# nreHieW/Eagle

Hardware: AMD Instinct MI355X
Metric: frames/sec end-to-end (detect+keypoint+homography) @1280x720 (higher is better)
Workload: dtype f32 (split: hi/lo binary16 pairs, 3 x fp16 MFMA per product, fp32 accumulate); detector (1.4 % of the FLOP): f32, exact v_mfma_f32_16x16x4_f32 chains

## Files before the change

### eagle_amd/csrc/conv.hip

```cpp
#include <algorithm>
#include <cmath>
#include <cstdlib>
#include <mutex>

#include "common.h"
#include "dmath.h"
#include "conv_internal.h"

namespace eagle {

static int f16_ps(int kc) { const int g = kc / 8; return kc * 2 + ((g % 2 == 0) ? 16 : 0); }
static int f16_ni(int ks, int kc) { return (ks * ks * (kc / 8) + 3) / 4; }

enum FormKind { GENERIC, WSTAT, ADIRECT };
enum StrideForm { S1, S2D, S2T };
enum WeightImage { W_F32, W_F16, W_F16_S2D, W_SPLIT, W_SPLIT_AD, W_SPLIT_S2D, W_SPLIT_M32 };
struct Form {
    int prec, variant, kind;
    int pw;
    int sform, rows, cols;
    int kc, nt, halo_bufs;
    int wimage;
    int grid_cap;
    ConvKernelGetter get;
};
static constexpr Form gen(int prec, int variant, int pw, int wimage, int kind = GENERIC) { return {prec, variant, kind, pw, S1, 0, 0, 0, 0, 0, wimage, 0, nullptr}; }
static constexpr Form ad(int prec, int variant, int sform, int rows, int cols, int nt, int halo_bufs, int wimage, ConvKernelGetter get, int grid_cap = 0)
{
    return {prec, variant, ADIRECT, 0, sform, rows, cols, prec == EAGLE_PREC_F16 ? 32 : 16, nt, halo_bufs, wimage, grid_cap, get};
}
static constexpr int F16 = EAGLE_PREC_F16, F32 = EAGLE_PREC_F32, F32S = EAGLE_PREC_F32S;
static constexpr Form g_forms[] = {
    gen(F32, 0, 4, W_F32), gen(F32, 3, 2, W_F32), gen(F32, 4, 1, W_F32),
    gen(F16, 0, 4, W_F16), gen(F16, 2, 4, W_F16), gen(F16, 3, 2, W_F16), gen(F16, 4, 1, W_F16), gen(F16, 6, 4, W_F16, WSTAT), gen(F16, 7, 2, W_F16, WSTAT),
    ad(F16, 8, S1, 4, 32, 12, 2, W_F16, conv_ad_kernel_s1_bn192), ad(F16, 9, S1, 8, 32, 6, 2, W_F16, conv_ad_kernel_s1_bn96),
    ad(F16, 10, S2D, 4, 32, 12, 2, W_F16_S2D, conv_ad_kernel_s2_bn192), ad(F16, 11, S2D, 8, 32, 6, 2, W_F16_S2D, conv_ad_kernel_s2_bn96),
    gen(F32S, 0, 4, W_SPLIT), gen(F32S, 3, 2, W_SPLIT), gen(F32S, 18, 6, W_SPLIT),
    ad(F32S, 8, S1, 4, 32, 12, 2, W_SPLIT_AD, conv_ad_split_kernel_bn192), ad(F32S, 9, S1, 8, 32, 6, 2, W_SPLIT_AD, conv_ad_split_kernel_bn96),
    ad(F32S, 10, S2D, 4, 32, 12, 2, W_SPLIT_S2D, conv_ad_split_kernel_s2_bn192), ad(F32S, 11, S2D, 8, 32, 6, 2, W_SPLIT_S2D, conv_ad_split_kernel_s2_bn96),
    ad(F32S, 12, S1, 8, 32, 3, 2, W_SPLIT_AD, conv_ad_split_kernel48), ad(F32S, 13, S1, 16, 32, 3, 1, W_SPLIT_AD, conv_ad_split_kernel48sb),
    ad(F32S, 19, S1, 16, 32, 3, 2, W_SPLIT_AD, conv_ad_split_kernel48ring, 256),
    ad(F32S, 14, S2T, 4, 32, 12, 1, W_SPLIT_AD, conv_ad_split_kernel_s2t_bn192), ad(F32S, 15, S2T, 4, 32, 6, 1, W_SPLIT_AD, conv_ad_split_kernel_s2t_bn96),
    ad(F32S, 21, S1, 4, 32, 12, 2, W_SPLIT_M32, conv_ad_split32_kernel_bn192), ad(F32S, 22, S1, 8, 32, 6, 2, W_SPLIT_M32, conv_ad_split32_kernel_bn96),
    ad(F32S, 23, S1, 2, 64, 12, 2, W_SPLIT_M32, conv_ad_split32_kernel_w64_bn192), ad(F32S, 24, S1, 4, 64, 6, 2, W_SPLIT_M32, conv_ad_split32_kernel_w64_bn96)};

static const Form* find_form(int precision, int variant)
{
    for (const Form& f : g_forms)
        if (f.prec == precision && f.variant == variant) return &f;
    return nullptr;
}
static const Form& form_of(int precision, const ConvConfig& c)
{
    const Form* f = find_form(precision, c.variant);
    if (!f) fail(EAGLE_E_NOKERNEL, "no conv kernel form: prec=%d variant=%d", precision, c.variant);
    return *f;
}
static int kind_of(int precision, const ConvConfig& c) { const Form* f = find_form(precision, c.variant); return f ? f->kind : -1; }

static size_t lds_bytes(int precision, const ConvConfig& c)
{
    const Form& f = form_of(precision, c);
    if (f.kind == ADIRECT) {
        int hpix, rec, strips;
        if (precision == EAGLE_PREC_F16) { hpix = f.sform == S2D ? (f.rows + 1) * 33 : (f.rows + 2) * 34; rec = 96; strips = 4 * 32 * 112; }
        else if (f.wimage == W_SPLIT_M32) { hpix = (f.rows + 2) * (f.cols + 2); rec = 80; strips = 4 * 32 * 128; }
        else { hpix = f.sform == S2T ? (2 * f.rows + 1) * 66 : (f.rows + 2) * 34; rec = 96; strips = 4 * 16 * 208; }
        const int slabs = ((hpix * rec + 1023) / 1024 + 3) / 4 * 4;
        return (size_t)f.halo_bufs * slabs * 1024 + strips;
    }
    const int th = 4 * f.pw / c.wx, tw = 16 * c.wx;
    const int hw = (tw - 1) * c.stride + c.ks, hh = (th - 1) * c.stride + c.ks;
    const int bn = c.nt * 16;
    if (precision == EAGLE_PREC_F16) {
        const size_t operands = (size_t)f16_ni(c.ks, c.kc) * 4 * bn * 16 + (size_t)hh * hw * f16_ps(c.kc);
        const size_t strips = (size_t)4 * f.pw * 16 * (bn * 2 + 16);
        return f.kind == WSTAT ? operands + strips + 16 : std::max(operands + 16, strips);
    }
    if (precision == EAGLE_PREC_F32S) {
        const size_t operands = (size_t)f16_ni(c.ks, c.kc) * 2 * 4 * bn * 16 + (size_t)hh * hw * f16_ps(2 * c.kc);
        const size_t strips = (size_t)4 * f.pw * 16 * (bn * 4 + 16);
        return std::max(operands + 16, strips);
    }
    return (size_t)c.ks * c.ks * (c.kc / 4) * 4 * bn * 4 + (size_t)hh * hw * (c.kc + 1) * 4;
}

size_t conv_lds_bytes(int precision, const ConvConfig& c) { return lds_bytes(precision, c); }
int conv_tiles_per_frame(int precision, const ConvConfig& c, int ho, int wo)
{
    const Form& f = form_of(precision, c);
    const int th = f.kind == ADIRECT ? f.rows : 4 * f.pw / c.wx, tw = f.kind == ADIRECT ? f.cols : 16 * c.wx;
    return ((wo + tw - 1) / tw) * ((ho + th - 1) / th);
}

static const Inst* generic_inst(int precision, const ConvConfig& c)
{
    for (auto part : {conv_inst_part0, conv_inst_part1, conv_inst_part2, conv_inst_part3, conv_inst_split0, conv_inst_split1, conv_inst_split2}) {
        int n = 0;
        const Inst* t = part(&n);
        for (int k = 0; k < n; ++k)
            if (t[k].prec == precision && t[k].ks == c.ks && t[k].s == c.stride && t[k].kc == c.kc && t[k].nt == c.nt && t[k].variant == c.variant) return &t[k];
    }
    return nullptr;
}
bool conv_supported(int precision, const ConvConfig& c)
{
    const Form* f = find_form(precision, c.variant);
    if (f && f->kind == ADIRECT) return c.ks == 3 && c.stride == (f->sform == S1 ? 1 : 2) && c.kc == f->kc && c.nt == f->nt;
    return f && generic_inst(precision, c);
}

struct Tuned { int ks, s, cin, cout, wo, kc, nt, wx, variant; };
static const Tuned g_tuned[] = {
#include "conv_tuned.inc"
    {0, 0, 0, 0, 0, 0, 0, 0, 0}};
static const Tuned g_tuned_f32[] = {
#include "conv_tuned_f32.inc"
    {0, 0, 0, 0, 0, 0, 0, 0, 0}};
static const Tuned g_tuned_split[] = {
#include "conv_tuned_split.inc"
    {0, 0, 0, 0, 0, 0, 0, 0, 0}};
static bool tuned_match(const Tuned& t, const ConvConfig& c, int wo, ConvConfig* q)
{
    if (t.ks != c.ks || t.s != c.stride || t.cin != c.cin || t.cout != c.cout_pad || t.wo != wo) return false;
    *q = c; q->kc = t.kc; q->nt = t.nt; q->wx = t.wx; q->variant = t.variant;
    return true;
}

static bool env_force(const char* name, int* a, int* b, int* c) { const char* f = getenv(name); return f && sscanf(f, "%d,%d,%d", a, b, c) == 3; }
static bool env_off(const char* name) { const char* e = getenv(name); return e && atoi(e) == 0; }

static const int g_nts[] = {6, 4, 3, 2, 1};
static ConvConfig with_ad(ConvConfig c, int kc, int v192, int v96)
{
    c.kc = kc;
    if (c.cout_pad % 192 == 0) { c.nt = 12; c.variant = v192; } else { c.nt = 6; c.variant = v96; }
    return c;
}

static ConvConfig choose_f32(ConvConfig c, int wo)
{
    ConvConfig q = c; q.kc = (c.cin < 16) ? 4 : 16;
    if (env_force("EAGLE_F32_FORCE", &q.nt, &q.wx, &q.variant) && (q.wx == 1 || q.wx == 2) && q.nt >= 1 && c.cout_pad % (16 * q.nt) == 0 &&
        conv_supported(EAGLE_PREC_F32, q) && lds_bytes(EAGLE_PREC_F32, q) <= 160 * 1024)
        return q;
    for (const Tuned& t : g_tuned_f32)
        if (tuned_match(t, c, wo, &q) && conv_supported(EAGLE_PREC_F32, q)) return q;
    c.nt = 1;
    for (int nt : g_nts)
        if (c.cout_pad % (16 * nt) == 0) { c.nt = nt; break; }
    c.kc = (c.cin < 16) ? 4 : 16;
    if (c.stride == 2 && c.ks == 3) {
        q = c; q.variant = 3;
        if (conv_supported(EAGLE_PREC_F32, q)) return q;
    }
    return c;
}

static ConvConfig choose_split(ConvConfig c, int wo, bool plain_epilogue)
{
    const int prec = EAGLE_PREC_F32S, cin = c.cin, cout = c.cout_pad;
    ConvConfig q = c;
    if (env_force("EAGLE_CONV_FORCE", &q.kc, &q.nt, &q.variant) && cin % q.kc == 0 && cout % (16 * q.nt) == 0 && conv_supported(prec, q)) {
        if (form_of(prec, q).pw == 6) q.wx = 3;
        if (lds_bytes(prec, q) <= 160 * 1024) return q;
    }
    if (plain_epilogue && c.ks == 3 && c.stride == 2 && cin % 48 == 0 && cout % 96 == 0) return with_ad(c, 16, 14, 15);
    if (!env_off("EAGLE_CONV_M32") && plain_epilogue && c.ks == 3 && c.stride == 1 && cin % 16 == 0 && cout % 96 == 0) return with_ad(c, 16, 21, wo > 32 ? 24 : 22);
    for (const Tuned& t : g_tuned_split)
        if (tuned_match(t, c, wo, &q)) {
            const Form* f = find_form(prec, q.variant);
            if (kind_of(prec, q) == ADIRECT && !(plain_epilogue && cin % (f->sform == S2D ? 16 : 48) == 0)) continue;
            if (conv_supported(prec, q) && lds_bytes(prec, q) <= 160 * 1024) return q;
        }
    if (plain_epilogue && c.ks == 3 && c.stride == 1 && cin % 48 == 0 && cout % 96 == 0) return with_ad(c, 16, 8, 9);
    static const int skcs[] = {32, 16, 8};
    long best = -1;
    c.nt = 1; c.kc = 8; c.variant = 0;
    for (int variant : {0, 3})
        for (int nt : g_nts) {
            if (cout % (16 * nt)) continue;
            for (int kc : skcs) {
                if (cin % kc) continue;
                ConvConfig t = c; t.nt = nt; t.kc = kc; t.variant = variant;
                if (!conv_supported(prec, t)) continue;
                if (lds_bytes(prec, t) > 80 * 1024) continue;
                const int pw = form_of(prec, t).pw;
                if (nt * pw > 12) continue;
                const long score = (long)nt * pw * 1000 + kc * 10 + (variant == 0 ? 1 : 0);
                if (score > best) { best = score; c.nt = nt; c.kc = kc; c.variant = variant; }
            }
        }
    return c;
}

static ConvConfig choose_f16(ConvConfig c, int wo, bool plain_epilogue, bool plain_one)
{
    const int prec = EAGLE_PREC_F16, cin = c.cin, cout = c.cout_pad;
    ConvConfig q = c;
    if (env_force("EAGLE_CONV_FORCE", &q.kc, &q.nt, &q.variant) && cin % q.kc == 0 && cout % (16 * q.nt) == 0 && conv_supported(prec, q) &&
        lds_bytes(prec, q) <= 160 * 1024 && (kind_of(prec, q) == WSTAT ? plain_one : kind_of(prec, q) == ADIRECT ? plain_epilogue : true))
        return q;
    if (plain_epilogue && c.ks == 3 && c.stride == 1 && cin % 32 == 0 && cout % 96 == 0) return with_ad(c, 32, 8, 9);
    if (plain_epilogue && c.ks == 3 && c.stride == 2 && cin % 8 == 0 && cin >= 32 && cout % 96 == 0) return with_ad(c, 32, 10, 11);
    for (const Tuned& t : g_tuned)
        if (tuned_match(t, c, wo, &q)) {
            if (kind_of(prec, q) == WSTAT && !plain_one) continue;
            if (conv_supported(prec, q) && lds_bytes(prec, q) <= 160 * 1024) return q;
        }
    static const int kcs[] = {64, 48, 32, 16, 8};
    long best = -1;
    c.nt = 1; c.kc = 8;
    for (int nt : g_nts) {
        if (cout % (16 * nt)) continue;
        for (int kc : kcs) {
            if (cin % kc) continue;
            ConvConfig t = c; t.nt = nt; t.kc = kc;
            if (!conv_supported(prec, t)) continue;
            if (lds_bytes(prec, t) > 80 * 1024) continue;
            const long score = (long)kc * nt * 1000 + kc;
            if (score > best) { best = score; c.nt = nt; c.kc = kc; }
        }
    }
    return c;
}

ConvConfig conv_choose(int precision, int ks, int stride, int cin_pad, int cout_pad, int wo, bool plain_epilogue, bool second_residual)
{
    ConvConfig c;
    c.ks = ks; c.stride = stride; c.cin = cin_pad; c.cout_pad = cout_pad;
    c.wx = (wo > 16) ? 2 : 1;
    if (precision == EAGLE_PREC_F32) return choose_f32(c, wo);
    if (precision == EAGLE_PREC_F32S) return choose_split(c, wo, plain_epilogue);
    return choose_f16(c, wo, plain_epilogue, plain_epilogue && !second_residual);
}

size_t conv_weight_elems(int precision, const ConvConfig& c)
{
    const int bn = c.nt * 16, nblk = c.cout_pad / bn, nch = c.cin / c.kc;
    switch (form_of(precision, c).wimage) {
    case W_F16_S2D: return (size_t)nblk * (4 * c.cin / 32) * 16 * bn * 8;
    case W_F16: return (size_t)nblk * nch * f16_ni(c.ks, c.kc) * 4 * bn * 8;
    case W_SPLIT_S2D: return (size_t)nblk * (4 * c.cin / 16) * 6 * 4 * bn * 8;
    case W_SPLIT_M32: return (size_t)nblk * (c.cin / 16) * 18 * (bn / 32) * 512;
    case W_SPLIT_AD: return (size_t)nblk * (c.cin / 16) * 14 * 4 * bn * 8;
    case W_SPLIT: return (size_t)nblk * nch * f16_ni(c.ks, c.kc) * 2 * 4 * bn * 8;
    default: return (size_t)nblk * nch * c.ks * c.ks * (c.kc / 4) * 4 * bn;
    }
}

void conv_tile_weights(int precision, const ConvConfig& c, const float* w, int cin_real, int cout_real, void* dst, float* descale)
{
    const int bn = c.nt * 16, nblk = c.cout_pad / bn, nch = c.cin / c.kc, taps = c.ks * c.ks, wimage = form_of(precision, c).wimage;
    auto W = [&](int tap, int ci, int co) -> float {
        return (ci < cin_real && co < cout_real) ? w[((size_t)tap * cin_real + ci) * cout_real + co] : 0.0f;
    };
    if (descale) *descale = 1.0f;
    if (precision == EAGLE_PREC_F32S) {
        float amax = 0.f;
        for (size_t k = 0; k < (size_t)taps * cin_real * cout_real; ++k) amax = std::max(amax, std::fabs(w[k]));
        int e = 0;
        if (amax > 0.f) (void)std::frexp(amax, &e);
        const int sw = 15 - e;
        const float scale = std::ldexp(1.0f, sw);
        if (descale) *descale = std::ldexp(1.0f, -(sw + 4));
        _Float16* d = (_Float16*)dst;
        if (wimage == W_SPLIT_S2D) {
            const int per_phase = c.cin / 16;
            for (int b = 0; b < nblk; ++b)
                for (int ch = 0; ch < 4 * per_phase; ++ch)
                    for (int k = 0; k < 6; ++k)
                        for (int qq = 0; qq < 4; ++qq)
                            for (int nn = 0; nn < bn; ++nn)
                                for (int j = 0; j < 8; ++j) {
                                    const int ph = ch / per_phase, c0 = (ch - ph * per_phase) * 16, ry = ph >> 1, rx = ph & 1;
                                    const int tp = k < 4 ? k : 2 * (k - 4) + (qq >> 1), tyy = tp >> 1, txx = tp & 1;
                                    const int ky = tyy == 0 ? (ry == 1 ? 0 : -1) : (ry == 0 ? 1 : 2), kx = txx == 0 ? (rx == 1 ? 0 : -1) : (rx == 0 ? 1 : 2);
                                    float v = 0.f;
                                    if (ky >= 0 && kx >= 0) v = W(ky * 3 + kx, c0 + (qq & 1) * 8 + j, b * bn + nn) * scale;
                                    const _Float16 hi = (_Float16)v;
                                    *d++ = k < 4 ? hi : (_Float16)(v - (float)hi);
                                }
            return;
        }
        if (wimage == W_SPLIT_M32) {
            for (int b = 0; b < nblk; ++b)
                for (int ch = 0; ch < c.cin / 16; ++ch)
                    for (int tap = 0; tap < 9; ++tap)
                        for (int part = 0; part < 2; ++part)
                            for (int mb = 0; mb < bn / 32; ++mb)
                                for (int l = 0; l < 64; ++l)
                                    for (int j = 0; j < 8; ++j) {
                                        const float v = W(tap, ch * 16 + (l >> 5) * 8 + j, b * bn + mb * 32 + (l & 31)) * scale;
                                        const _Float16 hi = (_Float16)v;
                                        *d++ = part == 0 ? hi : (_Float16)(v - (float)hi);
                                    }
            return;
        }
        if (wimage == W_SPLIT_AD) {
            for (int b = 0; b < nblk; ++b)
                for (int ch = 0; ch < c.cin / 16; ++ch)
                    for (int k = 0; k < 14; ++k)
                        for (int qq = 0; qq < 4; ++qq)
                            for (int nn = 0; nn < bn; ++nn)
                                for (int j = 0; j < 8; ++j) {
                                    const int tap = k < 9 ? k : 2 * (k - 9) + (qq >> 1);
                                    float v = 0.f;
                                    if (tap < 9) v = W(tap, ch * 16 + (qq & 1) * 8 + j, b * bn + nn) * scale;
                                    const _Float16 hi = (_Float16)v;
                                    *d++ = k < 9 ? hi : (_Float16)(v - (float)hi);
                                }
            return;
        }
        const int G = c.kc / 8, NGR = taps * G, NI = f16_ni(c.ks, c.kc);
        for (int b = 0; b < nblk; ++b)
            for (int ch = 0; ch < nch; ++ch)
                for (int i = 0; i < NI; ++i)
                    for (int part = 0; part < 2; ++part)
                        for (int qq = 0; qq < 4; ++qq)
                            for (int nn = 0; nn < bn; ++nn)
                                for (int j = 0; j < 8; ++j) {
                                    const int g = 4 * i + qq;
                                    float v = 0.f;
                                    if (g < NGR) { const int tap = g / G, cg = g % G; v = W(tap, ch * c.kc + cg * 8 + j, b * bn + nn) * scale; }
                                    const _Float16 hi = (_Float16)v;
                                    *d++ = part == 0 ? hi : (_Float16)(v - (float)hi);
                                }
        return;
    }
    if (wimage == W_F16_S2D) {
        _Float16* d = (_Float16*)dst;
        const int nch2 = 4 * c.cin / 32;
        for (int b = 0; b < nblk; ++b)
            for (int ch = 0; ch < nch2; ++ch)
                for (int g = 0; g < 16; ++g)
                    for (int nn = 0; nn < bn; ++nn)
                        for (int j = 0; j < 8; ++j) {
                            const int tp = g / 4, cg = g % 4, tyy = tp >> 1, txx = tp & 1;
                            const int sc = ch * 32 + cg * 8 + j, ph = sc / c.cin, ci = sc - ph * c.cin, ry = ph >> 1, rx = ph & 1;
                            const int ky = tyy == 0 ? (ry == 1 ? 0 : -1) : (ry == 0 ? 1 : 2), kx = txx == 0 ? (rx == 1 ? 0 : -1) : (rx == 0 ? 1 : 2);
                            *d++ = (_Float16)((ky < 0 || kx < 0) ? 0.f : W(ky * 3 + kx, ci, b * bn + nn));
                        }
        return;
    }
    if (precision == EAGLE_PREC_F16) {
        const int G = c.kc / 8, NGR = taps * G, NI = f16_ni(c.ks, c.kc);
        _Float16* d = (_Float16*)dst;
        for (int b = 0; b < nblk; ++b)
            for (int ch = 0; ch < nch; ++ch)
                for (int g = 0; g < NI * 4; ++g)
                    for (int nn = 0; nn < bn; ++nn)
                        for (int j = 0; j < 8; ++j) {
                            float v = 0.f;
                            if (g < NGR) {
                                const int tap = g / G, cg = g % G;
                                v = W(tap, ch * c.kc + cg * 8 + j, b * bn + nn);
                            }
                            *d++ = (_Float16)v;
                        }
    } else {
        const int CSTEPS = c.kc / 4;
        float* d = (float*)dst;
        for (int b = 0; b < nblk; ++b)
            for (int ch = 0; ch < nch; ++ch)
                for (int tap = 0; tap < taps; ++tap)
                    for (int cs = 0; cs < CSTEPS; ++cs)
                        for (int qq = 0; qq < 4; ++qq)
                            for (int nn = 0; nn < bn; ++nn) *d++ = W(tap, ch * c.kc + cs * 4 + qq, b * bn + nn);
    }
}

static std::mutex g_page_mutex;
static const void* conv_zero_page()
{
    static void* z[64] = {};
    int dev = 0;
    HIP_CHECK(hipGetDevice(&dev));
    std::lock_guard<std::mutex> g(g_page_mutex);
    if (!z[dev]) { HIP_CHECK(hipMalloc(&z[dev], 256)); HIP_CHECK(hipMemset(z[dev], 0, 256)); }
    return z[dev];
}
static void* conv_trash_page()
{
    static void* z[64] = {};
    int dev = 0;
    HIP_CHECK(hipGetDevice(&dev));
    std::lock_guard<std::mutex> g(g_page_mutex);
    if (!z[dev]) HIP_CHECK(hipMalloc(&z[dev], 8192));
    return z[dev];
}

void conv_launch(int precision, const ConvLaunch& L, hipStream_t s)
{
    const ConvConfig& c = L.cfg;
    if (!conv_supported(precision, c)) fail(EAGLE_E_NOKERNEL, "no conv kernel instance: prec=%d ks=%d s=%d kc=%d nt=%d", precision, c.ks, c.stride, c.kc, c.nt);
    const Form& f = form_of(precision, c);
    ConvArgs a;
    a.x = L.x.p; a.xcs = L.x.cs; a.xoff = L.x.off; a.N = L.x.n; a.H = L.x.h; a.W = L.x.w;
    a.w = L.w; a.bias = L.bias;
    a.y = L.y.p; a.ycs = L.y.cs; a.yoff = L.y.off; a.Ho = L.y.h; a.Wo = L.y.w;
    a.r1 = L.r1.p; a.r1cs = L.r1.cs; a.r1off = L.r1.off;
    a.r2 = L.r2.p; a.r2cs = L.r2.cs; a.r2off = L.r2.off;
    a.descale = L.descale;
    if (precision == EAGLE_PREC_F32S) {
        if (L.x.f32 != 2 || (L.r1.p && L.r1.f32 != 2) || (L.r2.p && L.r2.f32 != 2) || L.y.f32 != (L.out_f32 ? 1 : 2))
            fail(EAGLE_E_INVALID, "split conv: operand tensor formats do not match the family");
        a.xcs *= 2; a.xoff *= 2; a.r1cs *= 2; a.r1off *= 2; a.r2cs *= 2; a.r2off *= 2;
        if (!L.out_f32) { a.ycs *= 2; a.yoff *= 2; }
    }
    if (!a.r1 && a.r2) { a.r1 = a.r2; a.r1cs = a.r2cs; a.r1off = a.r2off; a.r2 = nullptr; }
    a.pre_act = L.pre_act; a.post_act = L.post_act; a.out_f32 = L.out_f32 || precision == EAGLE_PREC_F32;
    a.wx = c.wx;
    a.nchunks = c.cin / c.kc;
    a.zeros = conv_zero_page(); a.trash = conv_trash_page(); a.xcd = 0; a.gy = 1; a.stack = 0;
    a.am = L.am_slot ? *L.am_slot : nullptr; a.am_cs = c.cout_pad;
    a.sat = (L.sat_slot && precision == EAGLE_PREC_F32S) ? *L.sat_slot : nullptr;
    if (f.kind == ADIRECT) {
        if (a.out_f32 || a.pre_act != 0 || a.post_act > 1 || L.am_slot || (precision == EAGLE_PREC_F32S && c.cin % (f.wimage == W_SPLIT_AD ? 48 : 16)))
            fail(EAGLE_E_NOKERNEL, "A-direct conv needs 2-byte / split output, pre_act none, post_act in {none, ReLU} and, in the split family, Cin = 16 k (48 k for variants 8, 9 and 12 - 15)");
        if (f.sform == S2D) a.nchunks = 4 * c.cin / c.kc;
        a.tiles_x = (a.Wo + f.cols - 1) / f.cols; a.tiles_y = (a.Ho + f.rows - 1) / f.rows;
        a.gy = c.cout_pad / (c.nt * 16);
        const size_t lim = (size_t)1 << 31;
        if ((size_t)a.N * a.H * a.W * a.xcs * 2 >= lim || (size_t)a.N * a.Ho * a.Wo * std::max(std::max(a.ycs, a.r1 ? a.r1cs : 0), a.r2 ? a.r2cs : 0) * 2 >= lim)
            fail(EAGLE_E_INVALID, "fp16 conv: a tensor of %d frames reaches 2 GiB; use a smaller device batch", a.N);
        const int nres = (a.r1 ? 1 : 0) + (a.r2 ? 1 : 0);
        const int items = a.tiles_x * a.tiles_y * a.N * a.gy;
        const bool deep = items <= 256;
        for (bool d : {false, true}) ensure_max_dynamic_lds((const void*)f.get(nres, d), 160 * 1024);
        hipLaunchKernelGGL(f.get(nres, deep), dim3(f.grid_cap ? std::min(items, f.grid_cap) : items), dim3(256), lds_bytes(precision, c), s, a);
        HIP_CHECK(hipGetLastError());
        return;
    }
    const int th = 4 * f.pw / c.wx, tw = 16 * c.wx;
    a.tiles_x = (a.Wo + tw - 1) / tw; a.tiles_y = (a.Ho + th - 1) / th;
    if (precision == EAGLE_PREC_F32) {
        if (!env_off("EAGLE_F32_STACK") && c.stride == 1 && a.N > 1 && a.Ho == a.H) { a.stack = 1; a.tiles_y = (a.N * (a.Ho + 1) + th - 1) / th; }
        if ((size_t)a.N * a.H * a.W * a.xcs * 4 >= ((size_t)1 << 31)) fail(EAGLE_E_INVALID, "fp32 conv: the input tensor of %d frames reaches 2 GiB; use a smaller device batch", a.N);
    }
    const bool ws = f.kind == WSTAT;
    if (a.am && (!prec_is_f16_kernels(precision) || ws))
        fail(EAGLE_E_NOKERNEL, "fused heat-map maxima need the generic fp16 kernel");
    if (prec_is_f16_kernels(precision)) {
        const size_t lim = (size_t)1 << 31;
        const size_t cs_out = std::max(std::max(a.out_f32 ? 2 * a.ycs : a.ycs, a.r1 ? a.r1cs : 0), a.r2 ? a.r2cs : 0);
        if ((size_t)a.N * a.H * a.W * a.xcs * 2 >= lim || (size_t)a.N * a.Ho * a.Wo * cs_out * 2 >= lim)
            fail(EAGLE_E_INVALID, "fp16 conv: a tensor of %d frames reaches 2 GiB; use a smaller device batch", a.N);
    }
    const ConvKernel fn = generic_inst(precision, c)->fn;
    const size_t lds = lds_bytes(precision, c);
    ensure_max_dynamic_lds((const void*)fn, 160 * 1024);
    const int gy = c.cout_pad / (c.nt * 16);
    int gx = a.stack ? a.tiles_x * a.tiles_y : a.tiles_x * a.tiles_y * a.N;
    if (ws) {
        if (c.kc != c.cin || a.out_f32 || a.r2 || a.pre_act != 0 || a.post_act > 1 || (size_t)a.N * a.H * a.W * a.xcs * 2 >= (1ull << 31) || (size_t)a.N * a.Ho * a.Wo * std::max(a.ycs, a.r1 ? a.r1cs : 0) * 2 >= (1ull << 31))
            fail(EAGLE_E_NOKERNEL, "weight-stationary conv needs kc == cin, fp16 output, at most one residual, pre_act none, post_act in {none, ReLU} and tensors below 2 GiB (kc=%d cin=%d)", c.kc, c.cin);
        const int per_cu = (int)std::max<size_t>(1, std::min<size_t>(2, (160 * 1024) / lds));
        const int unit = 8 * gy;
        gx = std::max(unit, std::min((gx * gy + unit - 1) / unit * unit, 256 * per_cu / unit * unit));
    }
    a.gy = gy;
    a.xcd = (prec_is_f16_kernels(precision) && !ws && (c.ks == 3 || (c.ks == 1 && gy > 1))) ? 1 : 0;
    dim3 grid(gx, gy);
    if (a.xcd) grid = dim3(gx * gy, 1);
    if (ws) grid = dim3(gx, 1);
    hipLaunchKernelGGL(fn, grid, dim3(256), lds, s, a);
    HIP_CHECK(hipGetLastError());
}

}
```

### eagle_amd/csrc/conv_ad_split32.hip

```cpp
#include <algorithm>
#include <cstdlib>
#include <type_traits>

#include "common.h"
#include "dmath.h"
#include "conv_internal.h"

namespace eagle {

#include "conv_kernels.inc"
#include "conv_ad_split32.inc"

ConvKernel conv_ad_split32_kernel_bn192(int n_res, bool deep)
{
    static const ConvKernel fn[2][3] = {
        {conv_split_ad32_kernel<2, 2, 0>, conv_split_ad32_kernel<2, 2, 1>, conv_split_ad32_kernel<2, 2, 2>},
        {conv_split_ad32_kernel<2, 2, 0, 6>, conv_split_ad32_kernel<2, 2, 1, 6>, conv_split_ad32_kernel<2, 2, 2, 6>}};
    return fn[deep ? 1 : 0][res_slot(n_res)];
}

ConvKernel conv_ad_split32_kernel_bn96(int n_res, bool deep)
{
    static const ConvKernel fn[2][3] = {
        {conv_split_ad32_kernel<1, 4, 0>, conv_split_ad32_kernel<1, 4, 1>, conv_split_ad32_kernel<1, 4, 2>},
        {conv_split_ad32_kernel<1, 4, 0, 6>, conv_split_ad32_kernel<1, 4, 1, 6>, conv_split_ad32_kernel<1, 4, 2, 6>}};
    return fn[deep ? 1 : 0][res_slot(n_res)];
}

ConvKernel conv_ad_split32_kernel_w64_bn192(int n_res, bool deep)
{
    static const ConvKernel fn[2][3] = {
        {conv_split_ad32_kernel<2, 2, 0, 3, 2>, conv_split_ad32_kernel<2, 2, 1, 3, 2>, conv_split_ad32_kernel<2, 2, 2, 3, 2>},
        {conv_split_ad32_kernel<2, 2, 0, 6, 2>, conv_split_ad32_kernel<2, 2, 1, 6, 2>, conv_split_ad32_kernel<2, 2, 2, 6, 2>}};
    return fn[deep ? 1 : 0][res_slot(n_res)];
}

ConvKernel conv_ad_split32_kernel_w64_bn96(int n_res, bool deep)
{
    static const ConvKernel fn[2][3] = {
        {conv_split_ad32_kernel<1, 4, 0, 3, 2>, conv_split_ad32_kernel<1, 4, 1, 3, 2>, conv_split_ad32_kernel<1, 4, 2, 3, 2>},
        {conv_split_ad32_kernel<1, 4, 0, 6, 2>, conv_split_ad32_kernel<1, 4, 1, 6, 2>, conv_split_ad32_kernel<1, 4, 2, 6, 2>}};
    return fn[deep ? 1 : 0][res_slot(n_res)];
}

}
```

### eagle_amd/csrc/conv_ad_split32.inc

```
#ifndef EAGLE_CONV_AD_SPLIT32_INC
#define EAGLE_CONV_AD_SPLIT32_INC
#ifndef EAGLE_ABL_M32
#define EAGLE_ABL_M32 0
#endif
#ifndef EAGLE_M32_RES_NT
#define EAGLE_M32_RES_NT 1
#endif
#ifndef EAGLE_M32_SAUX
#define EAGLE_M32_SAUX (EAGLE_STORE_NT * 2 + EAGLE_M32_RES_NT * 4)
#endif
using f32x16 = __attribute__((ext_vector_type(16))) float;
#if EAGLE_ABL_M32 == 1 || EAGLE_ABL_M32 == 6
__device__ __forceinline__ f32x16 abl_m32_xor(const half8& a_, const half8& b_, f32x16 c_)
{
    const u32x4 ua = __builtin_bit_cast(u32x4, a_), ub = __builtin_bit_cast(u32x4, b_);
    c_[0] = __builtin_bit_cast(float, __builtin_bit_cast(unsigned, c_[0]) ^ ua[0] ^ ub[3]);
    return c_;
}
#define EAGLE_MFMA_M32(A_, B_, C_) abl_m32_xor(A_, B_, C_)
#else
#define EAGLE_MFMA_M32(A_, B_, C_) __builtin_amdgcn_mfma_f32_32x32x16_f16(A_, B_, C_, 0, 0, 0)
#endif
__device__ __forceinline__ void split_store4x(char* dhi, char* dlo, float v0, float v1, float v2, float v3)
{
    const float s0 = __builtin_amdgcn_fmed3f(v0 * SPLIT_SX, -65504.0f, 65504.0f), s1 = __builtin_amdgcn_fmed3f(v1 * SPLIT_SX, -65504.0f, 65504.0f),
                s2 = __builtin_amdgcn_fmed3f(v2 * SPLIT_SX, -65504.0f, 65504.0f), s3 = __builtin_amdgcn_fmed3f(v3 * SPLIT_SX, -65504.0f, 65504.0f);
    const half4 hi = {(_Float16)s0, (_Float16)s1, (_Float16)s2, (_Float16)s3};
    const half4 lo = {(_Float16)(s0 - (float)hi[0]), (_Float16)(s1 - (float)hi[1]), (_Float16)(s2 - (float)hi[2]), (_Float16)(s3 - (float)hi[3])};
    *(half4*)dhi = hi; *(half4*)dlo = lo;
}
template <int CQ, int PG, int RES, int RING = 3, int NRH = 1>
__global__ __launch_bounds__(256, 2) void conv_split_ad32_kernel(ConvArgs a)
{
    static_assert(CQ * PG == 4, "four waves per workgroup");
    static_assert(NRH == 1 || NRH == 2, "the wave's two pixel blocks: one above the other (1) or side by side (2)");
    static_assert(18 % RING == 0 && RING >= 3, "the weight ring holds a divisor of the 18 steps of a chunk");
    using rsrc_t = __amdgpu_buffer_rsrc_t;
    constexpr unsigned OOB = 0x80000000u;
    constexpr int MB = 3, NR = 2, NRV = NR / NRH, NW = 4, BN = CQ * 96, TH = NRV * PG, TW = 32 * NRH;
    constexpr int KSTEP = (BN / 32) * 1024;
    constexpr int PS = 80, SPC = 18, AHEAD = RING - 1;
    constexpr int HW_ = TW + 2, HPIX = (TH + 2) * HW_;
    constexpr int HSLABS = ((HPIX * PS + 1023) / 1024 + NW - 1) / NW * NW, HB = HSLABS * 1024, HK = HSLABS / NW;
    constexpr int RS = 32 * 4, STRIP = 32 * RS;
    extern __shared__ __attribute__((aligned(16))) char smem[];
    char* const Hb = smem;
    char* const strip = smem + 2 * HB + (threadIdx.x >> 6) * STRIP;
    const int tid = threadIdx.x, lane = tid & 63, wave = __builtin_amdgcn_readfirstlane(tid >> 6);
    const int cq = wave % CQ, pg = wave / CQ, kh = lane >> 5, lx = lane & 31;
    const int gy = a.gy, nitems = a.tiles_x * a.tiles_y * a.N * gy, nwg = gridDim.x;
    int item0, item_end;
    {
        const int b = blockIdx.x, xcd = b & 7, k = b >> 3;
        const int wgs_here = (nwg + 7 - xcd) >> 3;
        const int qn = nitems >> 3, rn = nitems & 7;
        const int x0 = xcd < rn ? xcd * (qn + 1) : rn * (qn + 1) + (xcd - rn) * qn;
        const int xc = qn + (xcd < rn ? 1 : 0);
        item0 = x0 + (int)((long)xc * k / wgs_here);
        item_end = x0 + (int)((long)xc * (k + 1) / wgs_here);
    }
    if (item0 >= item_end) return;
    const int nloc = item_end - item0, nch = a.nchunks, GC = nloc * nch;
    const rsrc_t xrs = __builtin_amdgcn_make_buffer_rsrc((void*)a.x, 0, 0x7FFFFFFF, 0x00020000);
    const rsrc_t wrs = __builtin_amdgcn_make_buffer_rsrc((void*)a.w, 0, 0x7FFFFFFF, 0x00020000);
    const rsrc_t rrs = __builtin_amdgcn_make_buffer_rsrc((void*)a.r1, 0, 0x7FFFFFFF, 0x00020000);
    const rsrc_t rrs2 = __builtin_amdgcn_make_buffer_rsrc((void*)a.r2, 0, 0x7FFFFFFF, 0x00020000);
    const rsrc_t yrs = __builtin_amdgcn_make_buffer_rsrc((void*)a.y, 0, 0x7FFFFFFF, 0x00020000);
    constexpr bool RECOMP = HK > 6;
    const int e0 = wave * 64 + lane;
    int hpk[RECOMP ? 1 : HK];
    if constexpr (!RECOMP) {
#pragma unroll
        for (int k = 0; k < HK; ++k) {
            const int e = e0 + NW * 64 * k;
            const int pix = e / 5, slot = e - pix * 5;
            const int hy = pix / HW_, hx = pix - hy * HW_;
            hpk[k] = (pix < HPIX && slot < 4) ? (hy | (hx << 8) | (((slot & 1) * 2 + (slot >> 1)) << 16)) : -1;
        }
    }
    const int bbase = ((pg * NRV) * HW_ + lx) * PS + kh * 16;
    const unsigned wlane = (unsigned)((cq * MB * 64 + lane) * 16);

    auto decode = [&](int item, int& n, int& ty, int& tx, int& nb) {
        int t = item / gy; nb = item - t * gy;
        tx = t % a.tiles_x; t /= a.tiles_x;
        ty = t % a.tiles_y; n = t / a.tiles_y;
    };
    int h_g = 0, h_ch = 0, h_item = item0;
    int h_iy0, h_ix0, h_gb;
    auto halo_origin = [&](int item) {
        int n, ty, tx, nb; decode(item, n, ty, tx, nb);
        h_iy0 = ty * TH - 1; h_ix0 = tx * TW - 1;
        h_gb = (((n * a.H + h_iy0) * a.W + h_ix0) * a.xcs + a.xoff) * 2;
    };
    halo_origin(h_item);
    auto issue_h_slab = [&](int k) {
        char* dst = Hb + (h_g & 1) * HB;
        const unsigned so = (EAGLE_ABL_M32 == 8) ? 0u : (unsigned)(h_ch * 32) * 2u;
        int hy, hx, unit; bool live;
        if constexpr (RECOMP) {
            int e = e0 + NW * 64 * k;
            asm volatile("" : "+v"(e));
            const int pix = (int)(((unsigned)e * 52429u) >> 18), slot = e - pix * 5;
            hy = HW_ == 34 ? (int)(((unsigned)pix * 1928u) >> 16) : (int)(((unsigned)pix * 993u) >> 16); hx = pix - hy * HW_;
            unit = (slot & 1) * 2 + (slot >> 1);
            live = pix < HPIX && slot < 4;
        } else {
            hy = hpk[k] & 0xFF; hx = (hpk[k] >> 8) & 0xFF; unit = (hpk[k] >> 16) & 7; live = hpk[k] >= 0;
        }
        const int iy = h_iy0 + hy, ix = h_ix0 + hx;
        const unsigned off = !(live && (unsigned)iy < (unsigned)a.H && (unsigned)ix < (unsigned)a.W) ? OOB
                             : (unsigned)(h_gb + ((hy * a.W + hx) * a.xcs + unit * 8) * 2);
        __builtin_amdgcn_raw_ptr_buffer_load_lds(xrs, (__attribute__((address_space(3))) void*)(dst + (wave + NW * k) * 1024), 16,
                                                 ((EAGLE_ABL_M32 == 3 || EAGLE_ABL_M32 == 6 || EAGLE_ABL_M32 == 7) && h_g > 0) ? OOB : off, so, 0, 0);
    };
    auto advance_h = [&]() {
        if (h_g + 1 >= GC) return;
        ++h_g;
        if (++h_ch == nch) { h_ch = 0; ++h_item; halo_origin(h_item); }
    };
    auto issue_h = [&]() {
#pragma unroll
        for (int k = 0; k < HK; ++k) issue_h_slab(k);
        advance_h();
    };
    issue_h();
    int gc = 0;
    for (int item = item0; item < item_end; ++item) {
        int n, ty, tx, nb; decode(item, n, ty, tx, nb);
        const int oy0 = ty * TH, ox0 = tx * TW;
        f32x16 acc[MB][NR];
#pragma unroll
        for (int i = 0; i < MB; ++i)
#pragma unroll
            for (int p = 0; p < NR; ++p)
#pragma unroll
                for (int r = 0; r < 16; ++r) acc[i][p][r] = 0.f;
        u32x4 A[RING][MB];
        unsigned wsrc = (unsigned)(nb * nch * SPC) * (unsigned)KSTEP;
        const unsigned wend = wsrc + (unsigned)(nch * SPC) * (unsigned)KSTEP;
        bool abl_a_done = false;
        auto load_a = [&](int slot) {
            const unsigned so = wsrc < wend ? wsrc : wend - KSTEP;
#pragma unroll
            for (int mb = 0; mb < MB; ++mb)
                if (!((EAGLE_ABL_M32 == 2 || EAGLE_ABL_M32 == 6 || EAGLE_ABL_M32 == 7) && abl_a_done)) A[slot][mb] = __builtin_amdgcn_raw_buffer_load_b128(wrs, wlane + mb * 1024, so, 0);
            wsrc += KSTEP;
        };
#pragma unroll
        for (int s = 0; s < AHEAD; ++s) load_a(s);
        abl_a_done = true;
        for (int ch = 0; ch < nch; ++ch, ++gc) {
            if constexpr (AHEAD * MB == 6) asm volatile("s_waitcnt vmcnt(6)" ::: "memory");
            else asm volatile("s_waitcnt vmcnt(15)" ::: "memory");
            static_assert(AHEAD * MB == 6 || AHEAD * MB == 15, "vmcnt literal");
            __builtin_amdgcn_s_barrier();
            issue_h();
            const char* hb = Hb + (gc & 1) * HB + bbase;
            half8 Bh[2][NR], Bl[2][NR];
            auto read_b = [&](int slot, int tap) {
                const int ky = tap / 3, kx = tap - ky * 3;
#pragma unroll
                for (int p = 0; p < NR; ++p) {
                    Bh[slot][p] = *(const half8*)(hb + ((p / NRH + ky) * HW_ + (p % NRH) * 32 + kx) * PS);
                    Bl[slot][p] = *(const half8*)(hb + ((p / NRH + ky) * HW_ + (p % NRH) * 32 + kx) * PS + 32);
                }
            };
            read_b(0, 0);
#pragma unroll
            for (int t = 0; t < 9; ++t) {
                const int bs = (EAGLE_ABL_M32 == 4 || EAGLE_ABL_M32 == 6) ? 0 : (t & 1);
                load_a((2 * t + AHEAD) % RING);
                if (t + 1 < 9 && !(EAGLE_ABL_M32 == 4 || EAGLE_ABL_M32 == 6)) read_b((t + 1) & 1, t + 1);
#pragma unroll
                for (int p = 0; p < NR; ++p)
#pragma unroll
                    for (int mb = 0; mb < MB; ++mb) acc[mb][p] = EAGLE_MFMA_M32((half8)A[(2 * t) % RING][mb], Bh[bs][p], acc[mb][p]);
#pragma unroll
                for (int p = 0; p < NR; ++p)
#pragma unroll
                    for (int mb = 0; mb < MB; ++mb) acc[mb][p] = EAGLE_MFMA_M32((half8)A[(2 * t) % RING][mb], Bl[bs][p], acc[mb][p]);
                __builtin_amdgcn_sched_barrier(0);
                load_a((2 * t + 1 + AHEAD) % RING);
#pragma unroll
                for (int p = 0; p < NR; ++p)
#pragma unroll
                    for (int mb = 0; mb < MB; ++mb) acc[mb][p] = EAGLE_MFMA_M32((half8)A[(2 * t + 1) % RING][mb], Bh[bs][p], acc[mb][p]);
                __builtin_amdgcn_sched_barrier(0);
            }
        }
        const int co0 = nb * BN + cq * 96;
        __builtin_amdgcn_sched_barrier(0);
        const float ds = a.descale;
        int pstrip[4], ppx[4];
#pragma unroll
        for (int i = 0; i < 4; ++i) {
            const int e = i * 64 + lane, px = e >> 3, u = e & 7;
            pstrip[i] = px * RS + ((u ^ (px & 7)) * 16);
            ppx[i] = px | (u << 8);
        }
        auto piece_off = [&](int pass, int i, int cs, int off) -> unsigned {
            const int row = pass / MB, mb = pass - row * MB;
            const int oy = oy0 + pg * NRV + row / NRH, ox2 = ox0 + (row % NRH) * 32 + (ppx[i] & 0xFF), u = ppx[i] >> 8;
            return (oy < a.Ho && ox2 < a.Wo) ? (unsigned)((((n * a.Ho + oy) * a.Wo + ox2) * cs + off + (co0 + mb * 32) * 2 + u * 8) * 2) : OOB;
        };
        float vmax = 0.0f;
        constexpr int NPASS = NR * MB, PB = (RES == 2 && NRH == 2) ? 2 : (RES == 2 || (RES == 1 && NRH == 2)) ? 3 : 6;
        u32x4 rres[RES >= 1 ? PB : 1][4], rres2[RES >= 2 ? PB : 1][4];
        char* const sp = strip + lx * RS + kh * 8;
        const int sw = (lx & 7) * 16;
        auto run_hi = [&](int j) -> char* { return sp + ((j * 32) ^ sw); };
        auto run_lo = [&](int j) -> char* { return sp + ((j * 32 + 16) ^ sw); };
#pragma unroll
        for (int pb0 = 0; pb0 < NPASS; pb0 += PB) {
            if (RES >= 1) {
#pragma unroll
                for (int h2 = 0; h2 < PB; ++h2)
#pragma unroll
                    for (int i = 0; i < 4; ++i) rres[h2][i] = __builtin_amdgcn_raw_buffer_load_b128(rrs, piece_off(pb0 + h2, i, a.r1cs, a.r1off), 0, (EAGLE_M32_SAUX & 4) ? 2 : 0);
            }
            if (RES >= 2) {
#pragma unroll
                for (int h2 = 0; h2 < PB; ++h2)
#pragma unroll
                    for (int i = 0; i < 4; ++i) rres2[h2][i] = __builtin_amdgcn_raw_buffer_load_b128(rrs2, piece_off(pb0 + h2, i, a.r2cs, a.r2off), 0, (EAGLE_M32_SAUX & 4) ? 2 : 0);
            }
#pragma unroll
            for (int h2 = 0; h2 < PB; ++h2) {
                const int pass = pb0 + h2, row = pass / MB, mb = pass - row * MB;
                if (RES >= 1) {
#pragma unroll
                    for (int i = 0; i < 4; ++i) *(u32x4*)(strip + pstrip[i]) = rres[h2][i];
                }
                float v[4][4];
#pragma unroll
                for (int j = 0; j < 4; ++j) {
                    const float4 bv = *(const float4*)(a.bias + co0 + mb * 32 + j * 8 + kh * 4);
                    v[j][0] = acc[mb][row][j * 4 + 0] * ds + bv.x; v[j][1] = acc[mb][row][j * 4 + 1] * ds + bv.y;
                    v[j][2] = acc[mb][row][j * 4 + 2] * ds + bv.z; v[j][3] = acc[mb][row][j * 4 + 3] * ds + bv.w;
                    if (RES >= 1) {
                        const half4 rh = *(const half4*)run_hi(j), rl = *(const half4*)run_lo(j);
#pragma unroll
                        for (int r = 0; r < 4; ++r) v[j][r] = ((float)rh[r] + (float)rl[r]) * SPLIT_RX + v[j][r];
                    }
                }
                if (RES >= 2) {
#pragma unroll
                    for (int i = 0; i < 4; ++i) *(u32x4*)(strip + pstrip[i]) = rres2[h2][i];
#pragma unroll
                    for (int j = 0; j < 4; ++j) {
                        const half4 rh = *(const half4*)run_hi(j), rl = *(const half4*)run_lo(j);
#pragma unroll
                        for (int r = 0; r < 4; ++r) v[j][r] = v[j][r] + ((float)rh[r] + (float)rl[r]) * SPLIT_RX;
                    }
                }
#pragma unroll
                for (int j = 0; j < 4; ++j) {
                    if (a.post_act == 1) {
#pragma unroll
                        for (int r = 0; r < 4; ++r) v[j][r] = v[j][r] > 0.f ? v[j][r] : 0.f;
                    }
                    split_store4x(run_hi(j), run_lo(j), v[j][0], v[j][1], v[j][2], v[j][3]);
                    vmax = split_absmax4(vmax, v[j][0], v[j][1], v[j][2], v[j][3]);
                }
#pragma unroll
                for (int i = 0; i < 4; ++i)
                    __builtin_amdgcn_raw_buffer_store_b128(*(const u32x4*)(strip + pstrip[i]), yrs, (EAGLE_ABL_M32 >= 5 && EAGLE_ABL_M32 <= 7) ? OOB : piece_off(pass, i, a.ycs, a.yoff), 0, EAGLE_M32_SAUX & 3);
            }
        }
        split_report(a.sat, n, vmax);
    }
}

#endif
```

### eagle_amd/csrc/conv_internal.h

```cpp
#pragma once
#include "common.h"

namespace eagle {

using half8 = __attribute__((ext_vector_type(8))) _Float16;
using half4 = __attribute__((ext_vector_type(4))) _Float16;
using f32x4 = __attribute__((ext_vector_type(4))) float;
using u32x4 = __attribute__((ext_vector_type(4))) unsigned int;
using u32x2 = __attribute__((ext_vector_type(2))) unsigned int;

struct ConvArgs {
    const void* x; int xcs, xoff; int N, H, W;
    const void* w; const float* bias;
    void* y; int ycs, yoff; int Ho, Wo;
    const void* r1; int r1cs, r1off;
    const void* r2; int r2cs, r2off;
    int pre_act, post_act, out_f32;
    int wx, tiles_x, tiles_y, nchunks;
    int gy;
    int stack;
    int xcd;
    ArgmaxPart* am;
    int am_cs;
    float descale;
    const void* zeros;
    void* trash;
    unsigned* sat;
};

struct BneckArgs {
    const void* x; int xcs, xoff; int N, H, W, nch1;
    const void *w1, *w2, *w3; const float *b1, *b2, *b3; float ds1, ds2, ds3;
    const void* r; int rcs, roff;
    void* y; int ycs, yoff;
    int tiles_x, tiles_y;
    unsigned* sat;
    unsigned long long* dbg;
};

typedef void (*ConvKernel)(ConvArgs);
struct Inst { int prec, ks, s, kc, nt, variant; ConvKernel fn; };
const Inst* conv_inst_part0(int* n); const Inst* conv_inst_part1(int* n); const Inst* conv_inst_part2(int* n); const Inst* conv_inst_part3(int* n);
const Inst* conv_inst_split0(int* n); const Inst* conv_inst_split1(int* n); const Inst* conv_inst_split2(int* n);
inline int res_slot(int n_res) { return n_res < 0 ? 0 : n_res > 2 ? 2 : n_res; }
typedef ConvKernel (*ConvKernelGetter)(int n_res, bool deep);
ConvKernel conv_ad_kernel_s1_bn192(int n_res, bool deep);
ConvKernel conv_ad_kernel_s1_bn96(int n_res, bool deep);
ConvKernel conv_ad_kernel_s2_bn192(int n_res, bool deep);
ConvKernel conv_ad_kernel_s2_bn96(int n_res, bool deep);
ConvKernel conv_ad_split_kernel_bn192(int n_res, bool deep);
ConvKernel conv_ad_split_kernel_bn96(int n_res, bool deep);
ConvKernel conv_ad_split_kernel_s2_bn192(int n_res, bool deep);
ConvKernel conv_ad_split_kernel_s2_bn96(int n_res, bool deep);
ConvKernel conv_ad_split_kernel_s2t_bn192(int n_res, bool deep);
ConvKernel conv_ad_split_kernel_s2t_bn96(int n_res, bool deep);
ConvKernel conv_ad_split_kernel48(int n_res, bool deep);
ConvKernel conv_ad_split_kernel48sb(int n_res, bool deep);
ConvKernel conv_ad_split_kernel48ring(int n_res, bool deep);
ConvKernel conv_ad_split32_kernel_bn192(int n_res, bool deep);
ConvKernel conv_ad_split32_kernel_bn96(int n_res, bool deep);
ConvKernel conv_ad_split32_kernel_w64_bn192(int n_res, bool deep);
ConvKernel conv_ad_split32_kernel_w64_bn96(int n_res, bool deep);

}
```

Baseline: 823.8.

## Add true stride-2 form of the M32 split direct conv kernel

```diff
diff --git a/eagle_amd/csrc/conv.hip b/eagle_amd/csrc/conv.hip
--- a/eagle_amd/csrc/conv.hip
+++ b/eagle_amd/csrc/conv.hip
@@ -42,7 +42,8 @@
     ad(F32S, 19, S1, 16, 32, 3, 2, W_SPLIT_AD, conv_ad_split_kernel48ring, 256),
     ad(F32S, 14, S2T, 4, 32, 12, 1, W_SPLIT_AD, conv_ad_split_kernel_s2t_bn192), ad(F32S, 15, S2T, 4, 32, 6, 1, W_SPLIT_AD, conv_ad_split_kernel_s2t_bn96),
     ad(F32S, 21, S1, 4, 32, 12, 2, W_SPLIT_M32, conv_ad_split32_kernel_bn192), ad(F32S, 22, S1, 8, 32, 6, 2, W_SPLIT_M32, conv_ad_split32_kernel_bn96),
-    ad(F32S, 23, S1, 2, 64, 12, 2, W_SPLIT_M32, conv_ad_split32_kernel_w64_bn192), ad(F32S, 24, S1, 4, 64, 6, 2, W_SPLIT_M32, conv_ad_split32_kernel_w64_bn96)};
+    ad(F32S, 23, S1, 2, 64, 12, 2, W_SPLIT_M32, conv_ad_split32_kernel_w64_bn192), ad(F32S, 24, S1, 4, 64, 6, 2, W_SPLIT_M32, conv_ad_split32_kernel_w64_bn96),
+    ad(F32S, 27, S2T, 4, 32, 12, 1, W_SPLIT_M32, conv_ad_split32_kernel_s2t_bn192), ad(F32S, 28, S2T, 4, 32, 6, 1, W_SPLIT_M32, conv_ad_split32_kernel_s2t_bn96)};
 
 static const Form* find_form(int precision, int variant)
 {
@@ -64,7 +65,9 @@
     if (f.kind == ADIRECT) {
         int hpix, rec, strips;
         if (precision == EAGLE_PREC_F16) { hpix = f.sform == S2D ? (f.rows + 1) * 33 : (f.rows + 2) * 34; rec = 96; strips = 4 * 32 * 112; }
-        else if (f.wimage == W_SPLIT_M32) { hpix = (f.rows + 2) * (f.cols + 2); rec = 80; strips = 4 * 32 * 128; }
+        else if (f.wimage == W_SPLIT_M32) {
+            hpix = f.sform == S2T ? (2 * f.rows + 1) * (2 * f.cols + 2) : (f.rows + 2) * (f.cols + 2); rec = 80; strips = 4 * 32 * 128;
+        }
         else { hpix = f.sform == S2T ? (2 * f.rows + 1) * 66 : (f.rows + 2) * 34; rec = 96; strips = 4 * 16 * 208; }
         const int slabs = ((hpix * rec + 1023) / 1024 + 3) / 4 * 4;
         return (size_t)f.halo_bufs * slabs * 1024 + strips;
@@ -166,6 +169,7 @@
         if (lds_bytes(prec, q) <= 160 * 1024) return q;
     }
     if (plain_epilogue && c.ks == 3 && c.stride == 2 && cin % 48 == 0 && cout % 96 == 0) return with_ad(c, 16, 14, 15);
+    if (plain_epilogue && c.ks == 3 && c.stride == 2 && cin % 16 == 0 && cout % 96 == 0) return with_ad(c, 16, 27, 28);
     if (!env_off("EAGLE_CONV_M32") && plain_epilogue && c.ks == 3 && c.stride == 1 && cin % 16 == 0 && cout % 96 == 0) return with_ad(c, 16, 21, wo > 32 ? 24 : 22);
     for (const Tuned& t : g_tuned_split)
         if (tuned_match(t, c, wo, &q)) {
diff --git a/eagle_amd/csrc/conv_ad_split32.hip b/eagle_amd/csrc/conv_ad_split32.hip
--- a/eagle_amd/csrc/conv_ad_split32.hip
+++ b/eagle_amd/csrc/conv_ad_split32.hip
@@ -43,4 +43,20 @@
     return fn[deep ? 1 : 0][res_slot(n_res)];
 }
 
+ConvKernel conv_ad_split32_kernel_s2t_bn192(int n_res, bool deep)
+{
+    static const ConvKernel fn[2][3] = {
+        {conv_split_ad32_kernel<2, 2, 0, 3, 1, true, 2, true>, conv_split_ad32_kernel<2, 2, 1, 3, 1, true, 2, true>, conv_split_ad32_kernel<2, 2, 2, 3, 1, true, 2, true>},
+        {conv_split_ad32_kernel<2, 2, 0, 6, 1, true, 2, true>, conv_split_ad32_kernel<2, 2, 1, 6, 1, true, 2, true>, conv_split_ad32_kernel<2, 2, 2, 6, 1, true, 2, true>}};
+    return fn[deep ? 1 : 0][res_slot(n_res)];
 }
+
+ConvKernel conv_ad_split32_kernel_s2t_bn96(int n_res, bool deep)
+{
+    static const ConvKernel fn[2][3] = {
+        {conv_split_ad32_kernel<1, 4, 0, 3, 1, true, 1, true>, conv_split_ad32_kernel<1, 4, 1, 3, 1, true, 1, true>, conv_split_ad32_kernel<1, 4, 2, 3, 1, true, 1, true>},
+        {conv_split_ad32_kernel<1, 4, 0, 6, 1, true, 1, true>, conv_split_ad32_kernel<1, 4, 1, 6, 1, true, 1, true>, conv_split_ad32_kernel<1, 4, 2, 6, 1, true, 1, true>}};
+    return fn[deep ? 1 : 0][res_slot(n_res)];
+}
+
+}
diff --git a/eagle_amd/csrc/conv_ad_split32.inc b/eagle_amd/csrc/conv_ad_split32.inc
--- a/eagle_amd/csrc/conv_ad_split32.inc
+++ b/eagle_amd/csrc/conv_ad_split32.inc
@@ -29,23 +29,25 @@
     const half4 lo = {(_Float16)(s0 - (float)hi[0]), (_Float16)(s1 - (float)hi[1]), (_Float16)(s2 - (float)hi[2]), (_Float16)(s3 - (float)hi[3])};
     *(half4*)dhi = hi; *(half4*)dlo = lo;
 }
-template <int CQ, int PG, int RES, int RING = 3, int NRH = 1>
+template <int CQ, int PG, int RES, int RING = 3, int NRH = 1, bool S2T = false, int NR = 2, bool SB = false>
 __global__ __launch_bounds__(256, 2) void conv_split_ad32_kernel(ConvArgs a)
 {
     static_assert(CQ * PG == 4, "four waves per workgroup");
     static_assert(NRH == 1 || NRH == 2, "the wave's two pixel blocks: one above the other (1) or side by side (2)");
+    static_assert(NR == 2 || (NR == 1 && NRH == 1), "the wave's pixel blocks: two, or one");
+    static_assert(!S2T || NRH == 1, "true stride 2: 32-column tiles");
     static_assert(18 % RING == 0 && RING >= 3, "the weight ring holds a divisor of the 18 steps of a chunk");
     using rsrc_t = __amdgpu_buffer_rsrc_t;
     constexpr unsigned OOB = 0x80000000u;
-    constexpr int MB = 3, NR = 2, NRV = NR / NRH, NW = 4, BN = CQ * 96, TH = NRV * PG, TW = 32 * NRH;
+    constexpr int MB = 3, NRV = NR / NRH, NW = 4, BN = CQ * 96, TH = NRV * PG, TW = 32 * NRH;
     constexpr int KSTEP = (BN / 32) * 1024;
     constexpr int PS = 80, SPC = 18, AHEAD = RING - 1;
-    constexpr int HW_ = TW + 2, HPIX = (TH + 2) * HW_;
+    constexpr int HPL = TW + 1, HW_ = S2T ? 2 * HPL : TW + 2, HPIX = (S2T ? 2 * TH + 1 : TH + 2) * HW_, ROWREC = S2T ? 2 * HW_ : HW_;
     constexpr int HSLABS = ((HPIX * PS + 1023) / 1024 + NW - 1) / NW * NW, HB = HSLABS * 1024, HK = HSLABS / NW;
     constexpr int RS = 32 * 4, STRIP = 32 * RS;
     extern __shared__ __attribute__((aligned(16))) char smem[];
     char* const Hb = smem;
-    char* const strip = smem + 2 * HB + (threadIdx.x >> 6) * STRIP;
+    char* const strip = smem + (SB ? 1 : 2) * HB + (threadIdx.x >> 6) * STRIP;
     const int tid = threadIdx.x, lane = tid & 63, wave = __builtin_amdgcn_readfirstlane(tid >> 6);
     const int cq = wave % CQ, pg = wave / CQ, kh = lane >> 5, lx = lane & 31;
     const int gy = a.gy, nitems = a.tiles_x * a.tiles_y * a.N * gy, nwg = gridDim.x;
@@ -67,6 +69,7 @@
     const rsrc_t rrs2 = __builtin_amdgcn_make_buffer_rsrc((void*)a.r2, 0, 0x7FFFFFFF, 0x00020000);
     const rsrc_t yrs = __builtin_amdgcn_make_buffer_rsrc((void*)a.y, 0, 0x7FFFFFFF, 0x00020000);
     constexpr bool RECOMP = HK > 6;
+    static_assert(!S2T || RECOMP, "the true stride-2 form decomposes its slabs at every request");
     const int e0 = wave * 64 + lane;
     int hpk[RECOMP ? 1 : HK];
     if constexpr (!RECOMP) {
@@ -78,7 +81,7 @@
             hpk[k] = (pix < HPIX && slot < 4) ? (hy | (hx << 8) | (((slot & 1) * 2 + (slot >> 1)) << 16)) : -1;
         }
     }
-    const int bbase = ((pg * NRV) * HW_ + lx) * PS + kh * 16;
+    const int bbase = ((pg * NRV) * ROWREC + lx) * PS + kh * 16;
     const unsigned wlane = (unsigned)((cq * MB * 64 + lane) * 16);
 
     auto decode = [&](int item, int& n, int& ty, int& tx, int& nb) {
@@ -90,12 +93,12 @@
     int h_iy0, h_ix0, h_gb;
     auto halo_origin = [&](int item) {
         int n, ty, tx, nb; decode(item, n, ty, tx, nb);
-        h_iy0 = ty * TH - 1; h_ix0 = tx * TW - 1;
+        h_iy0 = (S2T ? 2 : 1) * ty * TH - 1; h_ix0 = (S2T ? 2 : 1) * tx * TW - 1;
         h_gb = (((n * a.H + h_iy0) * a.W + h_ix0) * a.xcs + a.xoff) * 2;
     };
     halo_origin(h_item);
     auto issue_h_slab = [&](int k) {
-        char* dst = Hb + (h_g & 1) * HB;
+        char* dst = Hb + (SB ? 0 : (h_g & 1)) * HB;
         const unsigned so = (EAGLE_ABL_M32 == 8) ? 0u : (unsigned)(h_ch * 32) * 2u;
         int hy, hx, unit; bool live;
         if constexpr (RECOMP) {
@@ -105,6 +108,7 @@
             hy = HW_ == 34 ? (int)(((unsigned)pix * 1928u) >> 16) : (int)(((unsigned)pix * 993u) >> 16); hx = pix - hy * HW_;
             unit = (slot & 1) * 2 + (slot >> 1);
             live = pix < HPIX && slot < 4;
+            if constexpr (S2T) { const int pl = hx >= HPL ? 1 : 0; hx = 2 * (hx - HPL * pl) + pl; live = live && hx <= 2 * TW; }
         } else {
             hy = hpk[k] & 0xFF; hx = (hpk[k] >> 8) & 0xFF; unit = (hpk[k] >> 16) & 7; live = hpk[k] >= 0;
         }
@@ -124,7 +128,7 @@
         for (int k = 0; k < HK; ++k) issue_h_slab(k);
         advance_h();
     };
-    issue_h();
+    if constexpr (!SB) issue_h();
     int gc = 0;
     for (int item = item0; item < item_end; ++item) {
         int n, ty, tx, nb; decode(item, n, ty, tx, nb);
@@ -151,19 +155,27 @@
         for (int s = 0; s < AHEAD; ++s) load_a(s);
         abl_a_done = true;
         for (int ch = 0; ch < nch; ++ch, ++gc) {
-            if constexpr (AHEAD * MB == 6) asm volatile("s_waitcnt vmcnt(6)" ::: "memory");
-            else asm volatile("s_waitcnt vmcnt(15)" ::: "memory");
-            static_assert(AHEAD * MB == 6 || AHEAD * MB == 15, "vmcnt literal");
-            __builtin_amdgcn_s_barrier();
-            issue_h();
-            const char* hb = Hb + (gc & 1) * HB + bbase;
+            if constexpr (SB) {
+                __builtin_amdgcn_s_barrier();
+                issue_h();
+                asm volatile("s_waitcnt vmcnt(0)" ::: "memory");
+                __builtin_amdgcn_s_barrier();
+            } else {
+                if constexpr (AHEAD * MB == 6) asm volatile("s_waitcnt vmcnt(6)" ::: "memory");
+                else asm volatile("s_waitcnt vmcnt(15)" ::: "memory");
+                static_assert(AHEAD * MB == 6 || AHEAD * MB == 15, "vmcnt literal");
+                __builtin_amdgcn_s_barrier();
+                issue_h();
+            }
+            const char* hb = Hb + (SB ? 0 : (gc & 1)) * HB + bbase;
             half8 Bh[2][NR], Bl[2][NR];
             auto read_b = [&](int slot, int tap) {
                 const int ky = tap / 3, kx = tap - ky * 3;
+                const int tk = S2T ? ky * HW_ + (kx & 1) * HPL + (kx >> 1) : ky * HW_ + kx;
 #pragma unroll
                 for (int p = 0; p < NR; ++p) {
-                    Bh[slot][p] = *(const half8*)(hb + ((p / NRH + ky) * HW_ + (p % NRH) * 32 + kx) * PS);
-                    Bl[slot][p] = *(const half8*)(hb + ((p / NRH + ky) * HW_ + (p % NRH) * 32 + kx) * PS + 32);
+                    Bh[slot][p] = *(const half8*)(hb + ((p / NRH) * ROWREC + (p % NRH) * 32 + tk) * PS);
+                    Bl[slot][p] = *(const half8*)(hb + ((p / NRH) * ROWREC + (p % NRH) * 32 + tk) * PS + 32);
                 }
             };
             read_b(0, 0);
@@ -205,7 +217,9 @@
             return (oy < a.Ho && ox2 < a.Wo) ? (unsigned)((((n * a.Ho + oy) * a.Wo + ox2) * cs + off + (co0 + mb * 32) * 2 + u * 8) * 2) : OOB;
         };
         float vmax = 0.0f;
-        constexpr int NPASS = NR * MB, PB = (RES == 2 && NRH == 2) ? 2 : (RES == 2 || (RES == 1 && NRH == 2)) ? 3 : 6;
+        constexpr int NPASS = NR * MB, PB0 = (RES == 2 && NRH == 2) ? 2 : (RES == 2 || (RES == 1 && NRH == 2)) ? 3 : 6;
+        constexpr int PB = PB0 < NPASS ? PB0 : NPASS;
+        static_assert(NPASS % PB == 0, "whole groups of passes");
         u32x4 rres[RES >= 1 ? PB : 1][4], rres2[RES >= 2 ? PB : 1][4];
         char* const sp = strip + lx * RS + kh * 8;
         const int sw = (lx & 7) * 16;
diff --git a/eagle_amd/csrc/conv_internal.h b/eagle_amd/csrc/conv_internal.h
--- a/eagle_amd/csrc/conv_internal.h
+++ b/eagle_amd/csrc/conv_internal.h
@@ -61,5 +61,7 @@
 ConvKernel conv_ad_split32_kernel_bn96(int n_res, bool deep);
 ConvKernel conv_ad_split32_kernel_w64_bn192(int n_res, bool deep);
 ConvKernel conv_ad_split32_kernel_w64_bn96(int n_res, bool deep);
+ConvKernel conv_ad_split32_kernel_s2t_bn192(int n_res, bool deep);
+ConvKernel conv_ad_split32_kernel_s2t_bn96(int n_res, bool deep);
 
 }
```

Result: no change. 824.9 (median of 6 runs) (+0.1%).
